# iDC-NEU/NeutronStarLite

Hardware: NVIDIA H100
Metric: gcn_aggregated_edges_per_sec (higher is better)
Workload: dtype f32

## Files before the change

neutronstarlite_b200/csrc/nts_plan.cu:

```cuda
#include <cub/cub.cuh>
#include <cuda_bf16.h>

#include <algorithm>
#include <type_traits>
#include <vector>

#include "nts_common.cuh"

struct nts_gather_plan {
  uint32_t n_rows = 0;
  uint64_t n_edges = 0;
  uint32_t gather_rows = 0;
  int slabs = 1;
  uint32_t slab_rows = 0;
  uint2 *pairs = nullptr;
  uint32_t *voff = nullptr;
  std::vector<uint64_t> slab_edge;
  float *workspace = nullptr;
  size_t workspace_floats = 0;
  __nv_bfloat16 *workspace_bf16 = nullptr;
  size_t workspace_bf16_elems = 0;
  int hub_cols = 0, hub_rows = 0;
  uint32_t *hub_col_ids = nullptr;
  uint32_t *hub_row_ids = nullptr;
  uint32_t lda_c = 0, lda_r = 0;
  float *dense = nullptr;
  size_t dense_floats = 0;
  int last_grid = 0, last_launches = 0, last_k = 0, last_u = 0, last_outv = 0;
  float tuned_ms = 0.f;
};

namespace nts {

static int g_plan_u = 0, g_plan_minb = 0, g_plan_q = 0, g_plan_variant = 0;

__device__ __forceinline__ uint32_t plan_find_row(const uint32_t *__restrict__ off, uint32_t n_rows, uint32_t e) {
  uint32_t lo = 0, hi = n_rows;
  while (hi - lo > 1) {
    uint32_t mid = lo + ((hi - lo) >> 1);
    if (__ldg(off + mid) <= e)
      lo = mid;
    else
      hi = mid;
  }
  return lo;
}

__global__ void plan_keys_kernel(const uint32_t *__restrict__ off, const uint32_t *__restrict__ idx,
                                 const uint32_t *__restrict__ slot_of, uint32_t base, uint32_t n_rows, uint32_t n_edges,
                                 uint32_t slab_rows, uint32_t slabs, uint32_t *__restrict__ key,
                                 uint32_t *__restrict__ val) {
  for (uint64_t e = (uint64_t)blockIdx.x * blockDim.x + threadIdx.x; e < n_edges; e += (uint64_t)gridDim.x * blockDim.x) {
    const uint32_t r = plan_find_row(off, n_rows, (uint32_t)e);
    const uint32_t id = __ldg(idx + e);
    const uint32_t g = slot_of ? __ldg(slot_of + id) : id - base;
    uint32_t s = g / slab_rows;
    if (s >= slabs)
      s = slabs - 1;
    key[e] = s * n_rows + r;
    val[e] = (uint32_t)e;
  }
}

__global__ void plan_pairs_kernel(const uint32_t *__restrict__ perm, const uint32_t *__restrict__ idx,
                                  const float *__restrict__ w, const uint32_t *__restrict__ slot_of, uint32_t base,
                                  uint32_t n_edges, uint2 *__restrict__ pairs) {
  for (uint64_t i = (uint64_t)blockIdx.x * blockDim.x + threadIdx.x; i < n_edges; i += (uint64_t)gridDim.x * blockDim.x) {
    const uint32_t e = perm ? __ldg(perm + i) : (uint32_t)i;
    const uint32_t id = __ldg(idx + e);
    const uint32_t g = slot_of ? __ldg(slot_of + id) : id - base;
    const float wt = w ? __ldg(w + e) : 1.f;
    pairs[i] = make_uint2(g, __float_as_uint(wt));
  }
}

__global__ void plan_part_keys_kernel(const uint32_t *__restrict__ off, const uint32_t *__restrict__ idx,
                                      const uint32_t *__restrict__ slot_of, const float *__restrict__ w, uint32_t base,
                                      uint32_t index_add, uint32_t n_rows_part, uint32_t row_add, uint32_t n_edges,
                                      uint32_t e_off, uint32_t n_rows_total, uint32_t slab_rows, uint32_t slabs,
                                      uint32_t *__restrict__ key, uint32_t *__restrict__ val,
                                      uint2 *__restrict__ unsorted) {
  for (uint64_t e = (uint64_t)blockIdx.x * blockDim.x + threadIdx.x; e < n_edges; e += (uint64_t)gridDim.x * blockDim.x) {
    const uint32_t r = plan_find_row(off, n_rows_part, (uint32_t)e) + row_add;
    const uint32_t id = __ldg(idx + e);
    const uint32_t g = (slot_of ? __ldg(slot_of + id) : id - base) + index_add;
    uint32_t s = g / slab_rows;
    if (s >= slabs)
      s = slabs - 1;
    key[e_off + e] = s * n_rows_total + r;
    val[e_off + e] = e_off + (uint32_t)e;
    unsorted[e_off + e] = make_uint2(g, __float_as_uint(w ? __ldg(w + e) : 1.f));
  }
}
__global__ void plan_permute_pairs_kernel(const uint32_t *__restrict__ perm, const uint2 *__restrict__ unsorted,
                                          uint32_t n_edges, uint2 *__restrict__ pairs) {
  for (uint64_t i = (uint64_t)blockIdx.x * blockDim.x + threadIdx.x; i < n_edges; i += (uint64_t)gridDim.x * blockDim.x)
    pairs[i] = unsorted[__ldg(perm + i)];
}

template <class KeyT>
__global__ void plan_offsets_kernel(const KeyT *__restrict__ sorted_key, uint32_t n_edges, uint32_t n_keys,
                                    uint32_t *__restrict__ voff) {
  for (uint64_t k = (uint64_t)blockIdx.x * blockDim.x + threadIdx.x; k <= n_keys; k += (uint64_t)gridDim.x * blockDim.x) {
    uint32_t lo = 0, hi = n_edges;
    while (lo < hi) {
      uint32_t mid = lo + ((hi - lo) >> 1);
      if (__ldg(sorted_key + mid) < (KeyT)k)
        lo = mid + 1;
      else
        hi = mid;
    }
    voff[k] = lo;
  }
}

constexpr uint32_t kNoHub = 0xffffffffu;

__global__ void plan_ref_count_kernel(const uint32_t *__restrict__ idx, const uint32_t *__restrict__ slot_of,
                                      uint32_t base, uint32_t n_edges, uint32_t *__restrict__ cnt) {
  for (uint64_t e = (uint64_t)blockIdx.x * blockDim.x + threadIdx.x; e < n_edges; e += (uint64_t)gridDim.x * blockDim.x) {
    const uint32_t id = __ldg(idx + e);
    atomicAdd(cnt + (slot_of ? __ldg(slot_of + id) : id - base), 1u);
  }
}

__global__ void plan_hybrid_keys_kernel(const uint32_t *__restrict__ off, const uint32_t *__restrict__ idx,
                                        const uint32_t *__restrict__ slot_of, uint32_t base, uint32_t n_rows,
                                        uint32_t n_edges, uint32_t slab_rows, uint32_t slabs,
                                        const uint32_t *__restrict__ col_slot, const uint32_t *__restrict__ row_slot,
                                        uint32_t lda_c, uint64_t dc_cells, uint32_t lda_r, uint64_t *__restrict__ key,
                                        uint32_t *__restrict__ val) {
  const uint64_t n_keys = (uint64_t)slabs * n_rows;
  for (uint64_t e = (uint64_t)blockIdx.x * blockDim.x + threadIdx.x; e < n_edges; e += (uint64_t)gridDim.x * blockDim.x) {
    const uint32_t r = plan_find_row(off, n_rows, (uint32_t)e);
    const uint32_t id = __ldg(idx + e);
    const uint32_t g = slot_of ? __ldg(slot_of + id) : id - base;
    const uint32_t cs = __ldg(col_slot + g), rs = __ldg(row_slot + r);
    uint64_t k;
    if (cs != kNoHub) {
      k = n_keys + (uint64_t)cs * lda_c + r;
    } else if (rs != kNoHub) {
      k = n_keys + dc_cells + (uint64_t)g * lda_r + rs;
    } else {
      uint32_t s = g / slab_rows;
      if (s >= slabs)
        s = slabs - 1;
      k = (uint64_t)s * n_rows + r;
    }
    key[e] = k;
    val[e] = (uint32_t)e;
  }
}

__global__ void plan_cell_sum_kernel(const uint64_t *__restrict__ cell_key, const uint32_t *__restrict__ run_start,
                                     const uint32_t *__restrict__ run_len, uint32_t n_runs,
                                     const uint32_t *__restrict__ perm, const float *__restrict__ w, uint64_t n_keys,
                                     float *__restrict__ dense) {
  const uint32_t lane = threadIdx.x & 31;
  for (uint64_t run = ((uint64_t)blockIdx.x * blockDim.x + threadIdx.x) >> 5; run < n_runs;
       run += ((uint64_t)gridDim.x * blockDim.x) >> 5) {
    const uint32_t b = __ldg(run_start + run), n = __ldg(run_len + run);
    float s = 0.f;
    for (uint32_t j = lane; j < n; j += 32)
      s += w ? __ldg(w + __ldg(perm + b + j)) : 1.f;
#pragma unroll
    for (int o = 16; o > 0; o >>= 1)
      s += __shfl_xor_sync(0xffffffffu, s, o);
    if (lane == 0)
      dense[__ldg(cell_key + run) - n_keys] = s;
  }
}

__global__ void pad_rows_kernel(const float *__restrict__ src, float *__restrict__ dst, uint32_t n_rows, uint32_t F,
                                uint32_t ld) {
  const uint64_t total = (uint64_t)n_rows * ld;
  for (uint64_t i = (uint64_t)blockIdx.x * blockDim.x + threadIdx.x; i < total; i += (uint64_t)gridDim.x * blockDim.x) {
    const uint64_t r = i / ld;
    const uint32_t c = (uint32_t)(i - r * ld);
    dst[i] = c < F ? __ldg(src + r * F + c) : 0.f;
  }
// ... 337 lines not shown
  auto flush = [&](bool whole) {
    float *orow = out + (size_t)row * F;
#pragma unroll
    for (int k = 0; k < K; k++) {
      const uint32_t col = (c0 + k * 32) * 4;
      if (act[k] && col < F) {
        if (whole)
          flush_chunk<OUTV, false>(orow, col, F, acc[k]);
        else
          flush_chunk<OUTV, true>(orow, col, F, acc[k]);
      }
      acc[k] = make_float4(0.f, 0.f, 0.f, 0.f);
    }
  };
  auto advance = [&](uint32_t ee) {
    flush(row_started_inside);
    do {
      row++;
      row_end = __ldg(off + row + 1);
    } while (ee >= row_end);
    row_started_inside = true;
  };
  if (bulk_bytes)
    p_mbar_wait(bar, 0);
  const uint2 *sp = s_pair - cta_e_base;
  auto issue = [&](uint32_t e, uint32_t stage) {
    const uint32_t src_row = sp[e].x;
    p_mbar_expect_tx(sbar + stage, row_bytes);
    p_bulk_g2s(sbuf + (size_t)stage * tile_vecs, in + (size_t)src_row * ld4 + tile * tile_vecs, row_bytes, sbar + stage);
  };
  if (lane == 0)
    for (uint32_t s = 0; s < STAGES && e0 + s < e1; s++)
      issue(e0 + s, s);
  uint32_t stage = 0, parity = 0;
  for (uint32_t e = e0; e < e1; e++) {
    const float w = __uint_as_float(sp[e].y);
    p_mbar_wait(sbar + stage, parity);
    const float4 *b = sbuf + (size_t)stage * tile_vecs + lane;
    float4 v[K];
#pragma unroll
    for (int k = 0; k < K; k++)
      if (act[k])
        v[k] = b[k * 32];
    if (e >= row_end)
      advance(e);
#pragma unroll
    for (int k = 0; k < K; k++)
      if (act[k]) {
        acc[k].x = fmaf(w, v[k].x, acc[k].x);
        acc[k].y = fmaf(w, v[k].y, acc[k].y);
        acc[k].z = fmaf(w, v[k].z, acc[k].z);
        acc[k].w = fmaf(w, v[k].w, acc[k].w);
      }
    __syncwarp();
    if (lane == 0 && e + STAGES < e1)
      issue(e + STAGES, stage);
    if (++stage == STAGES) {
      stage = 0;
      parity ^= 1u;
    }
  }
  flush(row_started_inside && row_end <= e1);
}

template <int K, int STAGES, int OUTV, int MINB>
static int launch_planned_tma(nts_gather_plan *pl, const PlanShape &sh, const float4 *in, uint32_t ld4, float *out,
                              uint32_t F, uint32_t Q, cudaStream_t st);

struct PlanShape {
  int k, u, outv, minb, g;
  uint32_t tiles, tile_vecs;
};

template <class T, int K, int U, int OUTV, int MINB, int G = 1>
static int launch_planned(nts_gather_plan *pl, const PlanShape &sh, const T *in_rows, uint32_t ldc, float *out,
                          uint32_t F, uint32_t Q, cudaStream_t st) {
  auto kern = planned_gather_sum_kernel<T, K, U, OUTV, MINB, G>;
  const auto *in = reinterpret_cast<const typename GatherT<T>::chunk *>(in_rows);
  const size_t smem = 16 + ((size_t)kPlanWarps * G * Q + 4) * 8;
  NTS_CUDA_OK(cudaFuncSetAttribute(kern, cudaFuncAttributeMaxDynamicSharedMemorySize, (int)smem));
  pl->last_launches = 0;
  for (int s = 0; s < pl->slabs; s++) {
    const uint64_t eb = pl->slab_edge[s], ee = pl->slab_edge[s + 1];
    if (ee <= eb)
      continue;
    const uint64_t quanta = (ee - eb + Q - 1) / Q;
    const uint64_t blocks = (quanta * sh.tiles + kPlanWarps * G - 1) / (kPlanWarps * G);
    NTS_ARG_CHECK(blocks <= 0x7fffffffull, "aggregation grid too large");
    kern<<<(unsigned)blocks, kPlanWarps * 32, smem, st>>>(in, ldc, out, F, pl->pairs, pl->voff + (size_t)s * pl->n_rows,
                                                          pl->n_rows, (uint32_t)eb, (uint32_t)ee, Q, sh.tiles,
                                                          sh.tile_vecs);
    NTS_LAUNCH_CHECK();
    pl->last_grid = (int)blocks;
    pl->last_launches++;
  }
  return 0;
}

template <int K, int STAGES, int OUTV, int MINB>
static int launch_planned_tma(nts_gather_plan *pl, const PlanShape &sh, const float4 *in, uint32_t ld4, float *out,
                              uint32_t F, uint32_t Q, cudaStream_t st) {
  auto kern = planned_gather_sum_tma_kernel<K, STAGES, OUTV, MINB>;
  const uint32_t pair_bytes = (kPlanWarps * Q + 4) * 8;
  const uint32_t ring_bytes = 8u * STAGES + 8u * (STAGES & 1) + STAGES * sh.tile_vecs * 16u;
  const size_t smem = 16 + pair_bytes + (size_t)kPlanWarps * ring_bytes;
  NTS_ARG_CHECK(smem <= 227 * 1024, "row-staging ring does not fit shared memory");
  NTS_CUDA_OK(cudaFuncSetAttribute(kern, cudaFuncAttributeMaxDynamicSharedMemorySize, (int)smem));
  pl->last_launches = 0;
  for (int s = 0; s < pl->slabs; s++) {
    const uint64_t eb = pl->slab_edge[s], ee = pl->slab_edge[s + 1];
    if (ee <= eb)
      continue;
    const uint64_t quanta = (ee - eb + Q - 1) / Q;
    const uint64_t blocks = (quanta * sh.tiles + kPlanWarps - 1) / kPlanWarps;
    NTS_ARG_CHECK(blocks <= 0x7fffffffull, "aggregation grid too large");
    kern<<<(unsigned)blocks, kPlanWarps * 32, smem, st>>>(in, ld4, out, F, pl->pairs, pl->voff + (size_t)s * pl->n_rows,
                                                          pl->n_rows, (uint32_t)eb, (uint32_t)ee, Q, sh.tiles,
                                                          sh.tile_vecs, pair_bytes);
    NTS_LAUNCH_CHECK();
    pl->last_grid = (int)blocks;
    pl->last_launches++;
  }
  return 0;
}

#define NTS_PLAN_TMA_CASE(K_, S_, B_)                                                                               \
  if (sh.k == K_ && stages == S_ && sh.minb == B_) {                                                                \
    if (sh.outv == 4)                                                                                               \
      return launch_planned_tma<K_, S_, 4, B_>(pl, sh, in4, ld4, out, F, Q, st);                                    \
    if (sh.outv == 2)                                                                                               \
      return launch_planned_tma<K_, S_, 2, B_>(pl, sh, in4, ld4, out, F, Q, st);                                    \
    return launch_planned_tma<K_, S_, 1, B_>(pl, sh, in4, ld4, out, F, Q, st);                                      \
  }

#define NTS_PLAN_CASE_G(U_, B_, G_)                                                                                 \
  if (sh.k == 1 && sh.u == U_ && sh.minb == B_ && sh.g == G_) {                                                     \
    if (sh.outv == 4)                                                                                               \
      return launch_planned<T, 1, U_, 4, B_, G_>(pl, sh, in, ldc, out, F, Q, st);                                   \
    if (sh.outv == 2)                                                                                               \
      return launch_planned<T, 1, U_, 2, B_, G_>(pl, sh, in, ldc, out, F, Q, st);                                   \
    return launch_planned<T, 1, U_, 1, B_, G_>(pl, sh, in, ldc, out, F, Q, st);                                     \
  }

#define NTS_PLAN_CASE(K_, U_, B_)                                                                                   \
  if (sh.k == K_ && sh.u == U_ && sh.minb == B_) {                                                                  \
    if (sh.outv == 4)                                                                                               \
      return launch_planned<T, K_, U_, 4, B_>(pl, sh, in, ldc, out, F, Q, st);                                       \
    if (sh.outv == 2)                                                                                               \
      return launch_planned<T, K_, U_, 2, B_>(pl, sh, in, ldc, out, F, Q, st);                                       \
    return launch_planned<T, K_, U_, 1, B_>(pl, sh, in, ldc, out, F, Q, st);                                         \
  }

constexpr int kHubBM = 128, kHubBN = 128, kHubBK = 16, kHubThreads = 256;

__device__ __forceinline__ void p_cp_async16(void *smem_dst, const void *gmem_src, bool full) {
  asm volatile("cp.async.cg.shared.global [%0], [%1], 16, %2;" ::"r"(p_smem_u32(smem_dst)), "l"(gmem_src),
               "r"(full ? 16 : 0)
               : "memory");
}

template <class TB, int OUTV, bool SPLIT>
__global__ void __launch_bounds__(kHubThreads, 2)
    hub_block_gemm_kernel(const float *__restrict__ At, uint32_t lda, uint32_t M, uint32_t K, uint32_t k_split,
                          const TB *__restrict__ B, uint32_t ldb, const uint32_t *__restrict__ colmap,
                          float *__restrict__ out, uint32_t F, const uint32_t *__restrict__ rowmap, uint32_t m_tiles,
                          uint32_t n_tiles) {
  constexpr bool kBf16 = std::is_same<TB, __nv_bfloat16>::value;
  constexpr uint32_t kBV = 16 / sizeof(TB);
  __shared__ __align__(16) float As[2][kHubBK][kHubBM];
  __shared__ __align__(16) TB Bs[2][kHubBK][kHubBN];
  const uint32_t t = threadIdx.x;
  const uint32_t n_tile = blockIdx.x % n_tiles, rest = blockIdx.x / n_tiles;
  const uint32_t m0 = (rest % m_tiles) * kHubBM, n0 = n_tile * kHubBN;
  const uint32_t k_begin = (rest / m_tiles) * k_split;
  const uint32_t k_end = min(K, k_begin + k_split);
  if (k_begin >= k_end)
    return;
  const uint32_t n_kt = (k_end - k_begin + kHubBK - 1) / kHubBK;

  auto load = [&](uint32_t kt, int buf) {
#pragma unroll
    for (int i = 0; i < 2; i++) {
      const uint32_t c = t + i * kHubThreads, kk = c >> 5, c4 = (c & 31) * 4;
      const uint32_t k = k_begin + kt * kHubBK + kk;
      const bool a_ok = k < k_end && m0 + c4 < lda;
      p_cp_async16(&As[buf][kk][c4], a_ok ? At + (size_t)k * lda + m0 + c4 : At, a_ok);
    }
#pragma unroll
    for (int i = 0; i < (int)(kHubBK * kHubBN / kBV / kHubThreads); i++) {
      constexpr uint32_t kRowChunks = kHubBN / kBV;
      const uint32_t c = t + i * kHubThreads, kk = c / kRowChunks, cv = (c % kRowChunks) * kBV;
      const uint32_t k = k_begin + kt * kHubBK + kk;
      const bool b_ok = k < k_end && n0 + cv < ldb;
      const uint32_t brow = b_ok ? (colmap ? __ldg(colmap + k) : k) : 0;
      p_cp_async16(&Bs[buf][kk][cv], B + (size_t)brow * ldb + (b_ok ? n0 + cv : 0), b_ok);
    }
    asm volatile("cp.async.commit_group;" ::: "memory");
  };
  auto read_b4 = [&](int buf, int kk, uint32_t n) -> float4 {
    if constexpr (kBf16) {
      const uint2 u = *reinterpret_cast<const uint2 *>(&Bs[buf][kk][n]);
      return make_float4(__uint_as_float(u.x << 16), __uint_as_float(u.x & 0xffff0000u), __uint_as_float(u.y << 16),
                         __uint_as_float(u.y & 0xffff0000u));
    } else {
      return *reinterpret_cast<const float4 *>(&Bs[buf][kk][n]);
    }
  };

  const uint32_t tx = t & 15, ty = t >> 4;
  float acc[8][8];
#pragma unroll
  for (int i = 0; i < 8; i++)
#pragma unroll
    for (int j = 0; j < 8; j++)
      acc[i][j] = 0.f;

  load(0, 0);
  for (uint32_t kt = 0; kt < n_kt; kt++) {
    const int buf = kt & 1;
    if (kt + 1 < n_kt) {
      load(kt + 1, buf ^ 1);
      asm volatile("cp.async.wait_group 1;" ::: "memory");
    } else {
      asm volatile("cp.async.wait_group 0;" ::: "memory");
    }
    __syncthreads();
#pragma unroll
    for (int kk = 0; kk < kHubBK; kk++) {
      const float4 a0 = *reinterpret_cast<const float4 *>(&As[buf][kk][ty * 4]);
      const float4 a1 = *reinterpret_cast<const float4 *>(&As[buf][kk][64 + ty * 4]);
      const float4 b0 = read_b4(buf, kk, tx * 4);
      const float4 b1 = read_b4(buf, kk, 64 + tx * 4);
      const float a[8] = {a0.x, a0.y, a0.z, a0.w, a1.x, a1.y, a1.z, a1.w};
      const float b[8] = {b0.x, b0.y, b0.z, b0.w, b1.x, b1.y, b1.z, b1.w};
#pragma unroll
      for (int i = 0; i < 8; i++)
#pragma unroll
        for (int j = 0; j < 8; j++)
          acc[i][j] = fmaf(a[i], b[j], acc[i][j]);
    }
    __syncthreads();
  }

#pragma unroll
  for (int i = 0; i < 8; i++) {
    const uint32_t m = m0 + (i >> 2) * 64 + ty * 4 + (i & 3);
    if (m >= M)
      continue;
    float *orow = out + (size_t)(rowmap ? __ldg(rowmap + m) : m) * F;
#pragma unroll
    for (int j = 0; j < 2; j++) {
      const uint32_t col = n0 + j * 64 + tx * 4;
      if (col < F)
        flush_chunk<OUTV, SPLIT>(orow, col, F,
                                 make_float4(acc[i][j * 4], acc[i][j * 4 + 1], acc[i][j * 4 + 2], acc[i][j * 4 + 3]));
    }
  }
}

template <class TB, int OUTV>
static int launch_hub_blocks(nts_gather_plan *pl, const TB *in, uint32_t ldb, float *out, uint32_t F,
                             cudaStream_t st) {
  const uint32_t n_tiles = (F + kHubBN - 1) / kHubBN;
  if (pl->hub_cols) {
    const uint32_t m_tiles = (pl->n_rows + kHubBM - 1) / kHubBM;
    const uint64_t blocks = (uint64_t)m_tiles * n_tiles;
    NTS_ARG_CHECK(blocks <= 0x7fffffffull, "hub column block grid too large");
    hub_block_gemm_kernel<TB, OUTV, false><<<(unsigned)blocks, kHubThreads, 0, st>>>(
        pl->dense, pl->lda_c, pl->n_rows, (uint32_t)pl->hub_cols, (uint32_t)pl->hub_cols, in, ldb, pl->hub_col_ids, out,
        F, nullptr, m_tiles, n_tiles);
    NTS_LAUNCH_CHECK();
  }
  if (pl->hub_rows) {
    const uint32_t m_tiles = (pl->hub_rows + kHubBM - 1) / kHubBM;
    const uint32_t K = pl->gather_rows;
    const uint64_t want = (uint64_t)sm_count() * 2 * 4;
    uint64_t splits = (want + (uint64_t)m_tiles * n_tiles - 1) / ((uint64_t)m_tiles * n_tiles);
    uint32_t k_split = (uint32_t)((K + splits - 1) / splits);
    k_split = std::max<uint32_t>((k_split + kHubBK - 1) / kHubBK * kHubBK, 16 * kHubBK);
    splits = (K + k_split - 1) / k_split;
    hub_block_gemm_kernel<TB, OUTV, true><<<(unsigned)(splits * m_tiles * n_tiles), kHubThreads, 0, st>>>(
        pl->dense + (size_t)pl->hub_cols * pl->lda_c, pl->lda_r, (uint32_t)pl->hub_rows, K, k_split, in, ldb, nullptr,
        out, F, pl->hub_row_ids, m_tiles, n_tiles);
    NTS_LAUNCH_CHECK();
  }
  return 0;
}

template <class T>
static int run_gather(nts_gather_plan *pl, const T *in, uint32_t ld, float *output, uint32_t F, cudaStream_t st) {
  constexpr bool kBf16 = std::is_same<T, __nv_bfloat16>::value;
  PlanShape sh;
  const uint32_t ldc = ld / GatherT<T>::V;
  const uint32_t chunks = (ldc + 31) / 32;
  const uint32_t kmax = 5;
  sh.tiles = (chunks + kmax - 1) / kmax;
  sh.tile_vecs = (ldc + sh.tiles - 1) / sh.tiles;
  sh.k = (int)((sh.tile_vecs + 31) / 32);
  sh.tiles = (ldc + sh.tile_vecs - 1) / sh.tile_vecs;
  sh.outv = (F % 4 == 0 && aligned_to(output, 16)) ? 4 : ((F % 2 == 0 && aligned_to(output, 8)) ? 2 : 1);
  if (pl->hub_cols || pl->hub_rows) {
    const int rc = sh.outv == 4   ? launch_hub_blocks<T, 4>(pl, in, ld, output, F, st)
                   : sh.outv == 2 ? launch_hub_blocks<T, 2>(pl, in, ld, output, F, st)
                                  : launch_hub_blocks<T, 1>(pl, in, ld, output, F, st);
    if (rc)
      return rc;
  }
  sh.g = ldc <= 8 ? 4 : (ldc <= 16 ? 2 : 1);
  if (g_plan_variant == 1 || getenv("NTS_PLAN_NO_SUBWARP"))
    sh.g = 1;
  sh.minb = sh.k >= 3 ? 2 : (sh.k == 2 ? 3 : 4);
  sh.u = sh.k == 4 ? 2 : 4;
  if constexpr (kBf16) {
    sh.minb = sh.k >= 4 ? 2 : (sh.k >= 2 ? 3 : 4);
    sh.u = sh.k == 1 ? 4 : 2;
  }
  {
    static int env_read = 0;
    if (!env_read) {
      env_read = 1;
      if (const char *t = getenv("NTS_PLAN_TUNE"))
        sscanf(t, "%d,%d,%d", &g_plan_u, &g_plan_minb, &g_plan_q);
    }
    if (g_plan_u > 0)
      sh.u = g_plan_u;
    if (g_plan_minb > 0)
      sh.minb = g_plan_minb;
  }
  uint32_t Q = g_plan_q > 0 ? (uint32_t)g_plan_q : 512u / sh.g;
  if (g_plan_q <= 0) {
    const uint64_t per_slab = pl->slab_edge[pl->slabs] / (uint64_t)pl->slabs + 1;
    const uint64_t want_warps = (uint64_t)sm_count() * 64 * sh.g;
    while (Q > 32 && ((per_slab + Q - 1) / Q) * sh.tiles < want_warps)
      Q >>= 1;
  }
  Q = (Q + 31u) & ~31u;
  if (Q * sh.g > 1024)
    Q = (1024 / sh.g) & ~31u;
  pl->last_k = sh.k, pl->last_u = sh.u, pl->last_outv = sh.outv;
  float *out = output;
  if constexpr (kBf16) {
    NTS_PLAN_CASE_G(4, 4, 2)
    NTS_PLAN_CASE_G(4, 4, 4)
    NTS_PLAN_CASE_G(8, 2, 2)
    NTS_PLAN_CASE_G(8, 2, 4)
    if (sh.g != 1)
      return fail(-1, "no BF16 virtual-warp instantiation for this (U, occupancy) point", __FILE__, __LINE__);
    NTS_PLAN_CASE(1, 4, 4)
    NTS_PLAN_CASE(1, 8, 2)
    NTS_PLAN_CASE(2, 2, 3)
    NTS_PLAN_CASE(2, 4, 2)
    NTS_PLAN_CASE(3, 4, 2)
    NTS_PLAN_CASE(3, 2, 3)
    NTS_PLAN_CASE(3, 6, 1)
    NTS_PLAN_CASE(4, 2, 2)
    NTS_PLAN_CASE(4, 4, 2)
    NTS_PLAN_CASE(5, 2, 2)
    return fail(-1, "no BF16 planned-aggregation instantiation for this (chunks, U, occupancy) point", __FILE__,
                __LINE__);
  } else {
  const float4 *in4 = reinterpret_cast<const float4 *>(in);
  const uint32_t ld4 = ldc;
  if (g_plan_variant == 1) {
    const int stages = sh.u >= 8 ? 8 : (sh.u >= 4 ? 4 : 2);
    sh.minb = g_plan_minb > 0 ? g_plan_minb : (sh.k >= 4 ? 2 : 4);
    NTS_PLAN_TMA_CASE(1, 8, 4)
    NTS_PLAN_TMA_CASE(1, 4, 4)
    NTS_PLAN_TMA_CASE(1, 8, 3)
    NTS_PLAN_TMA_CASE(2, 4, 3)
    NTS_PLAN_TMA_CASE(2, 4, 2)
    NTS_PLAN_TMA_CASE(3, 4, 2)
    NTS_PLAN_TMA_CASE(4, 4, 2)
    NTS_PLAN_TMA_CASE(4, 2, 2)
    NTS_PLAN_TMA_CASE(5, 4, 2)
    NTS_PLAN_TMA_CASE(5, 2, 2)
    NTS_PLAN_TMA_CASE(5, 4, 1)
    NTS_PLAN_TMA_CASE(5, 8, 1)
    return fail(-1, "no TMA row-staging instantiation for this (chunks, stages, occupancy) point", __FILE__, __LINE__);
  }
  NTS_PLAN_CASE_G(4, 4, 2)
  NTS_PLAN_CASE_G(4, 4, 4)
  NTS_PLAN_CASE_G(8, 3, 2)
  NTS_PLAN_CASE_G(8, 3, 4)
  if (sh.g != 1)
    return fail(-1, "no virtual-warp instantiation for this (U, occupancy) point", __FILE__, __LINE__);
  NTS_PLAN_CASE(1, 8, 4)
  NTS_PLAN_CASE(1, 4, 4)
  NTS_PLAN_CASE(1, 8, 3)
  NTS_PLAN_CASE(1, 16, 2)
  NTS_PLAN_CASE(2, 4, 3)
  NTS_PLAN_CASE(2, 8, 2)
  NTS_PLAN_CASE(3, 4, 3)
  NTS_PLAN_CASE(3, 4, 2)
  NTS_PLAN_CASE(4, 2, 2)
  NTS_PLAN_CASE(4, 4, 2)
  NTS_PLAN_CASE(5, 2, 2)
  NTS_PLAN_CASE(5, 1, 3)
  NTS_PLAN_CASE(5, 2, 3)
  NTS_PLAN_CASE(5, 4, 1)
  NTS_PLAN_CASE(5, 4, 2)
  return fail(-1, "no planned-aggregation instantiation for this (chunks, U, occupancy) point", __FILE__, __LINE__);
  }
}

template <class E> static int ensure_workspace(E *&ws, size_t &have, size_t elems) {
  if (elems <= have)
    return 0;
  if (ws)
    NTS_CUDA_OK(cudaFree(ws));
  ws = nullptr;
  have = 0;
  NTS_CUDA_OK(cudaMalloc(reinterpret_cast<void **>(&ws), elems * sizeof(E)));
  have = elems;
  return 0;
}

static int run_plan(nts_gather_plan *pl, const float *input, float *output, uint32_t F, cudaStream_t st) {
  if (pl->n_rows == 0 || pl->n_edges == 0 || F == 0)
    return 0;
  NTS_ARG_CHECK(input && output, "null feature pointer");
  const uint32_t ld = (F + 3u) & ~3u;
  const float *in = input;
  if (ld != F || !aligned_to(input, 16)) {
    if (const int rc = ensure_workspace(pl->workspace, pl->workspace_floats, (size_t)pl->gather_rows * ld))
      return rc;
    const uint64_t total = (uint64_t)pl->gather_rows * ld;
    const unsigned blocks = (unsigned)std::min<uint64_t>((total + 255) / 256, (uint64_t)sm_count() * 32);
    pad_rows_kernel<<<blocks, 256, 0, st>>>(input, pl->workspace, pl->gather_rows, F, ld);
    NTS_LAUNCH_CHECK();
    in = pl->workspace;
  }
  return run_gather<float>(pl, in, ld, output, F, st);
}

int to_bf16_rows(const void *src, int dtype, uint32_t lds, void *dst, uint32_t n_rows, uint32_t F, uint32_t ld,
                 cudaStream_t st) {
  NTS_ARG_CHECK(dtype == NTS_DTYPE_F32 || dtype == NTS_DTYPE_BF16, "input dtype must be NTS_DTYPE_F32 or NTS_DTYPE_BF16");
  NTS_ARG_CHECK(ld % 8 == 0 && ld >= F && lds >= F && aligned_to(dst, 16), "bad BF16 row layout");
  if (!n_rows || !F)
    return 0;
  const uint64_t total = (uint64_t)n_rows * (ld / 8);
  const unsigned blocks = (unsigned)std::min<uint64_t>((total + 255) / 256, (uint64_t)sm_count() * 32);
  uint4 *d = static_cast<uint4 *>(dst);
  if (dtype == NTS_DTYPE_F32)
    bf16_rows_kernel<float><<<blocks, 256, 0, st>>>(static_cast<const float *>(src), lds, d, n_rows, F, ld);
  else
    bf16_rows_kernel<__nv_bfloat16><<<blocks, 256, 0, st>>>(static_cast<const __nv_bfloat16 *>(src), lds, d, n_rows,
                                                            F, ld);
  NTS_LAUNCH_CHECK();
  return 0;
}

int run_plan_bf16(nts_gather_plan *pl, const void *input, int dtype, uint32_t lds, float *output, uint32_t F,
                  cudaStream_t st) {
  NTS_ARG_CHECK(dtype == NTS_DTYPE_F32 || dtype == NTS_DTYPE_BF16, "input dtype must be NTS_DTYPE_F32 or NTS_DTYPE_BF16");
  NTS_ARG_CHECK(g_plan_variant == 0, "the TMA row-staging variant (nts_gather_plan_set_variant(1)) gathers FP32 rows only");
  if (pl->n_rows == 0 || pl->n_edges == 0 || F == 0)
    return 0;
  NTS_ARG_CHECK(input && output, "null feature pointer");
  NTS_ARG_CHECK(lds >= F, "row stride below the feature width");
  if (dtype == NTS_DTYPE_BF16 && lds % 8 == 0 && aligned_to(input, 16))
    return run_gather<__nv_bfloat16>(pl, static_cast<const __nv_bfloat16 *>(input), lds, output, F, st);
  const uint32_t ld = (F + 7u) & ~7u;
  if (const int rc = ensure_workspace(pl->workspace_bf16, pl->workspace_bf16_elems, (size_t)pl->gather_rows * ld))
    return rc;
  if (const int rc = to_bf16_rows(input, dtype, lds, pl->workspace_bf16, pl->gather_rows, F, ld, st))
    return rc;
  return run_gather<__nv_bfloat16>(pl, pl->workspace_bf16, ld, output, F, st);
}

}

using namespace nts;

extern "C" {

static int pick_slabs_for_rows(nts_vid_t gather_rows, uint64_t n_edges, nts_vid_t n_rows, uint64_t row_bytes,
                               uint64_t l2_budget_bytes) {
  if (!l2_budget_bytes)
    l2_budget_bytes = 16ull << 20;
  const uint64_t bytes = (uint64_t)gather_rows * row_bytes;
  uint64_t s = (bytes + l2_budget_bytes - 1) / l2_budget_bytes;
  const uint64_t by_degree = n_rows ? n_edges / ((uint64_t)n_rows * 16ull) : 1;
  if (s > by_degree)
    s = by_degree;
  if (s > 64)
    s = 64;
  return s < 1 ? 1 : (int)s;
}

int nts_gather_plan_pick_slabs(nts_vid_t gather_rows, uint64_t n_edges, nts_vid_t n_rows, nts_vid_t feature_size,
                               uint64_t l2_budget_bytes) {
  return pick_slabs_for_rows(gather_rows, n_edges, n_rows, ((feature_size + 3ull) & ~3ull) * 4ull, l2_budget_bytes);
}

static bool hub_counts(const nts_vid_t *offsets, const nts_vid_t *indices, const nts_vid_t *slot_of, nts_vid_t base,
                       uint32_t n_rows, uint32_t E, uint32_t gather_rows, std::vector<uint32_t> &col_cnt,
                       std::vector<uint32_t> &seg, cudaStream_t st) {
  uint32_t *cnt = nullptr;
  std::vector<uint32_t> off(n_rows + 1);
  col_cnt.assign(gather_rows, 0);
  const unsigned blocks = (unsigned)std::min<uint64_t>(((uint64_t)E + 255) / 256, (uint64_t)sm_count() * 32);
  bool ok = cudaMalloc(reinterpret_cast<void **>(&cnt), (size_t)gather_rows * 4) == cudaSuccess &&
            cudaMemsetAsync(cnt, 0, (size_t)gather_rows * 4, st) == cudaSuccess;
  if (ok && E) {
    plan_ref_count_kernel<<<blocks, 256, 0, st>>>(indices, slot_of, base, E, cnt);
    count_launch();
  }
  ok = ok && cudaMemcpyAsync(col_cnt.data(), cnt, (size_t)gather_rows * 4, cudaMemcpyDeviceToHost, st) == cudaSuccess &&
       cudaMemcpyAsync(off.data(), offsets, ((size_t)n_rows + 1) * 4, cudaMemcpyDeviceToHost, st) == cudaSuccess &&
       cudaStreamSynchronize(st) == cudaSuccess;
  cudaFree(cnt);
  seg.resize(n_rows);
  for (uint32_t r = 0; r < n_rows; r++)
    seg[r] = off[r + 1] - off[r];
  return ok;
}

static std::vector<uint32_t> top_ids(const std::vector<uint32_t> &cnt, size_t h) {
  std::vector<uint32_t> ids(cnt.size());
  for (size_t i = 0; i < ids.size(); i++)
    ids[i] = (uint32_t)i;
  h = std::min(h, ids.size());
  std::partial_sort(ids.begin(), ids.begin() + h, ids.end(),
                    [&](uint32_t a, uint32_t b) { return cnt[a] != cnt[b] ? cnt[a] > cnt[b] : a < b; });
  ids.resize(h);
  return ids;
}

static bool build_hybrid(nts_gather_plan *pl, const nts_vid_t *offsets, const nts_vid_t *indices, const float *weight,
                         const nts_vid_t *slot_of, nts_vid_t index_base, int n_hub_cols, int n_hub_rows,
                         cudaStream_t st) {
  const uint32_t E = (uint32_t)pl->n_edges, n_rows = pl->n_rows, G = pl->gather_rows;
  std::vector<uint32_t> col_cnt, seg;
  if (!hub_counts(offsets, indices, slot_of, index_base, n_rows, E, G, col_cnt, seg, st))
    return false;
  const std::vector<uint32_t> cols = top_ids(col_cnt, (size_t)n_hub_cols), rows = top_ids(seg, (size_t)n_hub_rows);
  pl->hub_cols = (int)cols.size();
  pl->hub_rows = (int)rows.size();
  pl->lda_c = (n_rows + 3u) & ~3u;
  pl->lda_r = ((uint32_t)pl->hub_rows + 3u) & ~3u;
  const uint64_t dc_cells = (uint64_t)pl->hub_cols * pl->lda_c;
  pl->dense_floats = dc_cells + (pl->hub_rows ? (uint64_t)G * pl->lda_r : 0);
  std::vector<uint32_t> col_slot(G, kNoHub), row_slot(n_rows, kNoHub);
  for (size_t i = 0; i < cols.size(); i++)
    col_slot[cols[i]] = (uint32_t)i;
  for (size_t i = 0; i < rows.size(); i++)
    row_slot[rows[i]] = (uint32_t)i;

  const uint64_t n_keys = (uint64_t)pl->slabs * n_rows;
  int bits = 1;
  while (bits < 64 && (1ull << bits) < n_keys + pl->dense_floats)
    bits++;
  uint64_t *key_in = nullptr, *key_out = nullptr;
  uint32_t *val_in = nullptr, *val_out = nullptr, *d_col_slot = nullptr, *d_row_slot = nullptr, *d_runs = nullptr;
// ... 193 lines not shown
  if (total >= 0xffffffffull)
    return bad("merged edge count must fit uint32 offsets");
  if (n_slabs < 1 || gather_rows == 0)
    n_slabs = 1;
  if ((uint64_t)n_slabs * n_rows >= 0xffffffffull)
    return bad("slabs * rows must fit 32-bit segment keys");
  nts_gather_plan *pl = new nts_gather_plan();
  pl->n_rows = n_rows;
  pl->n_edges = total;
  pl->gather_rows = gather_rows;
  pl->slabs = n_slabs;
  pl->slab_rows = gather_rows ? (gather_rows + n_slabs - 1) / n_slabs : 1;
  pl->slab_edge.assign(n_slabs + 1, 0);
  if (n_rows == 0 || total == 0)
    return pl;
  const uint32_t E = (uint32_t)total, n_keys = (uint32_t)n_slabs * n_rows;
  uint32_t *key_in = nullptr, *key_out = nullptr, *val_in = nullptr, *val_out = nullptr;
  uint2 *unsorted = nullptr;
  void *tmp = nullptr;
  size_t tmp_bytes = 0;
  int bits = 1;
  while (bits < 32 && (1ull << bits) < (uint64_t)n_keys)
    bits++;
  bool ok = cudaMalloc(reinterpret_cast<void **>(&pl->pairs), (size_t)E * sizeof(uint2)) == cudaSuccess &&
            cudaMalloc(reinterpret_cast<void **>(&pl->voff), ((size_t)n_keys + 1) * sizeof(uint32_t)) == cudaSuccess &&
            cudaMalloc(reinterpret_cast<void **>(&unsorted), (size_t)E * sizeof(uint2)) == cudaSuccess &&
            cudaMalloc(reinterpret_cast<void **>(&key_in), (size_t)E * 4) == cudaSuccess &&
            cudaMalloc(reinterpret_cast<void **>(&key_out), (size_t)E * 4) == cudaSuccess &&
            cudaMalloc(reinterpret_cast<void **>(&val_in), (size_t)E * 4) == cudaSuccess &&
            cudaMalloc(reinterpret_cast<void **>(&val_out), (size_t)E * 4) == cudaSuccess &&
            cub::DeviceRadixSort::SortPairs(nullptr, tmp_bytes, key_in, key_out, val_in, val_out, (int64_t)E, 0, bits, st) ==
                cudaSuccess &&
            cudaMalloc(&tmp, tmp_bytes ? tmp_bytes : 16) == cudaSuccess;
  uint32_t e_off = 0;
  for (int k = 0; k < n_parts && ok; k++) {
    const nts_plan_part &pt = parts[k];
    if (!pt.n_edges)
      continue;
    const unsigned blocks = (unsigned)std::min<uint64_t>((pt.n_edges + 255) / 256, (uint64_t)sm_count() * 32);
    plan_part_keys_kernel<<<blocks, 256, 0, st>>>(pt.offsets, pt.indices, pt.slot_of, pt.weight, pt.index_base,
                                                  pt.index_add, pt.n_rows, pt.row_add, (uint32_t)pt.n_edges, e_off, n_rows,
                                                  pl->slab_rows, (uint32_t)n_slabs, key_in, val_in, unsorted);
    count_launch();
    e_off += (uint32_t)pt.n_edges;
  }
  if (ok)
    ok = cub::DeviceRadixSort::SortPairs(tmp, tmp_bytes, key_in, key_out, val_in, val_out, (int64_t)E, 0, bits, st) ==
         cudaSuccess;
  if (ok) {
    const unsigned blocks = (unsigned)std::min<uint64_t>(((uint64_t)E + 255) / 256, (uint64_t)sm_count() * 32);
    plan_permute_pairs_kernel<<<blocks, 256, 0, st>>>(val_out, unsorted, E, pl->pairs);
    count_launch();
    const unsigned kb = (unsigned)std::min<uint64_t>(((uint64_t)n_keys + 256) / 256, (uint64_t)sm_count() * 32);
    plan_offsets_kernel<uint32_t><<<kb, 256, 0, st>>>(key_out, E, n_keys, pl->voff);
    count_launch();
    std::vector<uint32_t> h(n_slabs + 1);
    ok = cudaStreamSynchronize(st) == cudaSuccess;
    for (int s = 0; s <= n_slabs && ok; s++)
      ok = cudaMemcpy(&h[s], pl->voff + (size_t)s * n_rows, 4, cudaMemcpyDeviceToHost) == cudaSuccess;
    for (int s = 0; s <= n_slabs; s++)
      pl->slab_edge[s] = h[s];
  }
  if (ok)
    ok = cudaStreamSynchronize(st) == cudaSuccess && cudaGetLastError() == cudaSuccess;
  cudaFree(key_in), cudaFree(key_out), cudaFree(val_in), cudaFree(val_out), cudaFree(tmp), cudaFree(unsorted);
  if (!ok) {
    fail(-1, "nts_gather_plan_create_parts: device allocation or preprocessing failed", __FILE__, __LINE__);
    cudaFree(pl->pairs), cudaFree(pl->voff);
    delete pl;
    return nullptr;
  }
  return pl;
}

nts_gather_plan *nts_plan_create_parts_typed(const nts_plan_part *parts, int n_parts, nts_vid_t n_rows,
                                             nts_vid_t gather_rows, int n_slabs, nts_vid_t feature_size, int bf16,
                                             void *stream) {
  if (!parts || n_parts < 1) {
    fail(-1, "no plan parts", __FILE__, __LINE__);
    return nullptr;
  }
  cudaStream_t st = as_stream(stream);
  if (n_slabs >= 1)
    return build_plan_parts(parts, n_parts, n_rows, gather_rows, n_slabs, st);
  uint64_t total = 0;
  for (int k = 0; k < n_parts; k++)
    total += parts[k].n_edges;
  const uint64_t row_bytes = bf16 ? ((feature_size + 7ull) & ~7ull) * 2ull : ((feature_size + 3ull) & ~3ull) * 4ull;
  const int s_max = pick_slabs_for_rows(gather_rows, total, n_rows, row_bytes, 16ull << 20);
  nts_gather_plan *best = build_plan_parts(parts, n_parts, n_rows, gather_rows, 1, st);
  if (!best || s_max <= 1 || total == 0 || feature_size == 0)
    return best;
  float *x = nullptr, *y = nullptr;
  cudaEvent_t e0 = nullptr, e1 = nullptr;
  const size_t xb = (size_t)gather_rows * feature_size * (bf16 ? 2 : sizeof(float)),
               yb = (size_t)n_rows * feature_size * sizeof(float);
  bool ok = cudaMalloc(reinterpret_cast<void **>(&x), xb) == cudaSuccess &&
            cudaMalloc(reinterpret_cast<void **>(&y), yb) == cudaSuccess &&
            cudaMemsetAsync(x, 0, xb, st) == cudaSuccess && cudaMemsetAsync(y, 0, yb, st) == cudaSuccess &&
            cudaEventCreate(&e0) == cudaSuccess && cudaEventCreate(&e1) == cudaSuccess;
  auto time_plan = [&](nts_gather_plan *pl, float *ms) -> bool {
    *ms = 1e30f;
    for (int it = 0; it < 3; it++) {
      float t = 0.f;
      if (cudaEventRecord(e0, st) != cudaSuccess ||
          (bf16 ? run_plan_bf16(pl, x, NTS_DTYPE_BF16, feature_size, y, feature_size, st)
                : run_plan(pl, x, y, feature_size, st)) != 0 ||
          cudaEventRecord(e1, st) != cudaSuccess || cudaEventSynchronize(e1) != cudaSuccess ||
          cudaEventElapsedTime(&t, e0, e1) != cudaSuccess)
        return false;
      if (it > 0 && t < *ms)
        *ms = t;
    }
    return true;
  };
  float best_ms = 0.f;
  ok = ok && time_plan(best, &best_ms);
  for (int s = 2; ok; s *= 2) {
    const int cand = s > s_max ? s_max : s;
    nts_gather_plan *pl = build_plan_parts(parts, n_parts, n_rows, gather_rows, cand, st);
    float ms = 0.f;
    if (!pl || !time_plan(pl, &ms)) {
      nts_gather_plan_destroy(pl);
      break;
    }
    if (ms < best_ms) {
      nts_gather_plan_destroy(best);
      best = pl;
      best_ms = ms;
    } else {
      nts_gather_plan_destroy(pl);
      if (ms > 1.1f * best_ms)
        break;
    }
    if (cand == s_max)
      break;
  }
  cudaFree(x), cudaFree(y);
  if (e0)
    cudaEventDestroy(e0);
  if (e1)
    cudaEventDestroy(e1);
  best->tuned_ms = best_ms;
  return best;
}

nts_gather_plan *nts_gather_plan_create_parts(const nts_plan_part *parts, int n_parts, nts_vid_t n_rows,
                                              nts_vid_t gather_rows, int n_slabs, nts_vid_t feature_size, void *stream) {
  return nts_plan_create_parts_typed(parts, n_parts, n_rows, gather_rows, n_slabs, feature_size, 0, stream);
}

float nts_gather_plan_tuned_ms(const nts_gather_plan *pl) { return pl ? pl->tuned_ms : 0.f; }

static constexpr double kHubFloor = 0.05;
static constexpr int kHubMax = 512;

static nts_gather_plan *create_tuned(const nts_vid_t *offsets, const nts_vid_t *indices, const float *weight,
                                     const nts_vid_t *slot_of, nts_vid_t index_base, nts_vid_t n_rows, uint64_t n_edges,
                                     nts_vid_t gather_rows, nts_vid_t feature_size, bool bf16, void *stream) {
  cudaStream_t st = as_stream(stream);
  const uint64_t row_bytes = bf16 ? ((feature_size + 7ull) & ~7ull) * 2ull : ((feature_size + 3ull) & ~3ull) * 4ull;
  const int s_max = pick_slabs_for_rows(gather_rows, n_edges, n_rows, row_bytes, 16ull << 20);
  const char *hub_env = getenv("NTS_PLAN_HUBS");
  const bool try_hubs = !(hub_env && strcmp(hub_env, "0") == 0) && n_rows > 0 && gather_rows > 0;
  nts_gather_plan *best = nts_gather_plan_create(offsets, indices, weight, slot_of, index_base, n_rows, n_edges,
                                                 gather_rows, 1, stream);
  if (!best || (s_max <= 1 && !try_hubs) || n_edges == 0 || feature_size == 0)
    return best;
  float *x = nullptr, *y = nullptr;
  cudaEvent_t e0 = nullptr, e1 = nullptr;
  const size_t xb = (size_t)gather_rows * feature_size * (bf16 ? 2 : sizeof(float)),
               yb = (size_t)n_rows * feature_size * sizeof(float);
  bool ok = cudaMalloc(reinterpret_cast<void **>(&x), xb) == cudaSuccess &&
            cudaMalloc(reinterpret_cast<void **>(&y), yb) == cudaSuccess &&
            cudaMemsetAsync(x, 0, xb, st) == cudaSuccess && cudaMemsetAsync(y, 0, yb, st) == cudaSuccess &&
            cudaEventCreate(&e0) == cudaSuccess && cudaEventCreate(&e1) == cudaSuccess;
  auto run_one = [&](nts_gather_plan *pl) {
    return bf16 ? run_plan_bf16(pl, x, NTS_DTYPE_BF16, feature_size, y, feature_size, st)
                : run_plan(pl, x, y, feature_size, st);
  };
  auto time_plan = [&](nts_gather_plan *pl, float *ms) -> bool {
    *ms = 1e30f;
    for (int it = 0; it < 3; it++) {
      float t = 0.f;
      if (cudaEventRecord(e0, st) != cudaSuccess || run_one(pl) != 0 ||
          cudaEventRecord(e1, st) != cudaSuccess || cudaEventSynchronize(e1) != cudaSuccess ||
          cudaEventElapsedTime(&t, e0, e1) != cudaSuccess)
        return false;
      if (it > 0 && t < *ms)
        *ms = t;
    }
    return true;
  };
  float best_ms = 0.f;
  ok = ok && time_plan(best, &best_ms);
  auto consider = [&](int s, int hc, int hr, float *ms) -> int {
    nts_gather_plan *pl = nts_gather_plan_create_hybrid(offsets, indices, weight, slot_of, index_base, n_rows, n_edges,
                                                        gather_rows, s, hc, hr, stream);
    if (!pl || !time_plan(pl, ms)) {
      nts_gather_plan_destroy(pl);
      return -1;
    }
    if (*ms < best_ms) {
      nts_gather_plan_destroy(best);
      best = pl;
      best_ms = *ms;
      return 1;
    }
    nts_gather_plan_destroy(pl);
    return 0;
  };
  for (int s = 2; ok && s_max > 1; s *= 2) {
    const int cand = s > s_max ? s_max : s;
    float ms = 0.f;
    const int r = consider(cand, 0, 0, &ms);
    if (r < 0 || (r == 0 && ms > 1.1f * best_ms))
      break;
    if (cand == s_max)
      break;
  }
  if (ok && try_hubs) {
    std::vector<uint32_t> col_cnt, seg;
    ok = hub_counts(offsets, indices, slot_of, index_base, n_rows, (uint32_t)n_edges, gather_rows, col_cnt, seg, st);
    int n_c = 0, n_r = 0;
    for (uint32_t c : col_cnt)
      n_c += c > kHubFloor * n_rows;
    for (uint32_t s : seg)
      n_r += s > kHubFloor * gather_rows;
    const int plain_slabs = best->slabs;
    float ms = 0.f;
    for (int c = 32; ok && c <= std::min(n_c, kHubMax); c *= 2)
      if (consider(best->slabs, c, 0, &ms) != 1)
        break;
    for (int r = 32; ok && r <= std::min(n_r, kHubMax); r *= 2)
      if (consider(best->slabs, best->hub_cols, r, &ms) != 1)
        break;
    if (best->hub_cols || best->hub_rows) {
      const int hc = best->hub_cols, hr = best->hub_rows;
      for (int s : {plain_slabs / 2, std::min(plain_slabs * 2, s_max)})
        if (s >= 1 && s != plain_slabs && s != best->slabs)
          consider(s, hc, hr, &ms);
    }
  }
  cudaFree(x), cudaFree(y);
  if (e0)
    cudaEventDestroy(e0);
  if (e1)
    cudaEventDestroy(e1);
  best->tuned_ms = best_ms;
  return best;
}

nts_gather_plan *nts_gather_plan_create_tuned(const nts_vid_t *offsets, const nts_vid_t *indices, const float *weight,
                                              const nts_vid_t *slot_of, nts_vid_t index_base, nts_vid_t n_rows,
                                              uint64_t n_edges, nts_vid_t gather_rows, nts_vid_t feature_size,
                                              void *stream) {
  return create_tuned(offsets, indices, weight, slot_of, index_base, n_rows, n_edges, gather_rows, feature_size, false,
                      stream);
}

nts_gather_plan *nts_gather_plan_create_tuned_bf16(const nts_vid_t *offsets, const nts_vid_t *indices,
                                                   const float *weight, const nts_vid_t *slot_of, nts_vid_t index_base,
                                                   nts_vid_t n_rows, uint64_t n_edges, nts_vid_t gather_rows,
                                                   nts_vid_t feature_size, void *stream) {
  return create_tuned(offsets, indices, weight, slot_of, index_base, n_rows, n_edges, gather_rows, feature_size, true,
                      stream);
}

int nts_gather_plan_destroy(nts_gather_plan *pl) {
  if (!pl)
    return 0;
  cudaFree(pl->pairs);
  cudaFree(pl->voff);
  cudaFree(pl->workspace);
  cudaFree(pl->workspace_bf16);
  cudaFree(pl->dense);
  cudaFree(pl->hub_col_ids);
  cudaFree(pl->hub_row_ids);
  delete pl;
  return 0;
}

int nts_gather_plan_slabs(const nts_gather_plan *pl) { return pl ? pl->slabs : 0; }

int nts_gather_plan_hubs(const nts_gather_plan *pl, int *cols, int *rows) {
  NTS_ARG_CHECK(pl != nullptr, "null plan");
  if (cols)
    *cols = pl->hub_cols;
  if (rows)
    *rows = pl->hub_rows;
  return 0;
}

uint64_t nts_gather_plan_bytes(const nts_gather_plan *pl) {
  if (!pl)
    return 0;
  return pl->n_edges * 8ull + ((uint64_t)pl->slabs * pl->n_rows + 1) * 4ull + pl->workspace_floats * 4ull +
         pl->workspace_bf16_elems * 2ull + pl->dense_floats * 4ull + ((uint64_t)pl->hub_cols + pl->hub_rows) * 4ull;
}

int nts_gather_plan_last_launch(const nts_gather_plan *pl, int *launches, int *grid, int *k, int *u, int *outv) {
  NTS_ARG_CHECK(pl != nullptr, "null plan");
  if (launches)
    *launches = pl->last_launches;
  if (grid)
    *grid = pl->last_grid;
  if (k)
    *k = pl->last_k;
  if (u)
    *u = pl->last_u;
  if (outv)
    *outv = pl->last_outv;
  return 0;
}

int nts_gather_plan_run(nts_gather_plan *pl, const float *input, float *output, nts_vid_t feature_size, void *stream) {
  NTS_ARG_CHECK(pl != nullptr, "null plan");
  return run_plan(pl, input, output, feature_size, as_stream(stream));
}

int nts_gather_plan_run_bf16(nts_gather_plan *pl, const void *input, int input_dtype, float *output,
                             nts_vid_t feature_size, void *stream) {
  NTS_ARG_CHECK(pl != nullptr, "null plan");
  return run_plan_bf16(pl, input, input_dtype, feature_size, output, feature_size, as_stream(stream));
}

int nts_gather_plan_set_variant(int variant) {
  NTS_ARG_CHECK(variant == 0 || variant == 1, "variant must be 0 (register staging) or 1 (TMA row staging)");
  g_plan_variant = variant;
  return 0;
}

int nts_gather_plan_set_tuning(int u, int min_blocks, int edges_per_warp) {
  NTS_ARG_CHECK(u >= 0 && min_blocks >= 0 && edges_per_warp >= 0 && edges_per_warp <= 4096, "bad tuning point");
  g_plan_u = u;
  g_plan_minb = min_blocks;
  g_plan_q = edges_per_warp;
  return 0;
}

}
```

Before: 14.56 billion.

## Use 3xTF32 tensor-core MMA for hub GEMM, overlap hub rows on side stream

Replaces the FP32 SIMT outer-product inner loop of the hub block GEMM with mma.sync m16n8k8 TF32 instructions, using hi/lo splitting (3xTF32, or 2x for bf16 inputs) to keep near-FP32 accuracy. Shared-memory tiles gain row padding to reduce bank conflicts. The hub-row GEMM now runs on a separate non-blocking stream, forked and joined with events, so it can overlap the sparse gather launches. The hub selection floor and cap are also loosened so more hub columns and rows become dense. The extra MMA passes per tile and the changed stream dependencies add risk.

```diff
diff --git a/neutronstarlite_b200/csrc/nts_plan.cu b/neutronstarlite_b200/csrc/nts_plan.cu
--- a/neutronstarlite_b200/csrc/nts_plan.cu
+++ b/neutronstarlite_b200/csrc/nts_plan.cu
@@ -26,6 +26,9 @@
   uint32_t lda_c = 0, lda_r = 0;
   float *dense = nullptr;
   size_t dense_floats = 0;
+  cudaStream_t row_stream = nullptr;
+  cudaEvent_t row_fork = nullptr, row_join = nullptr;
+  bool row_forked = false;
   int last_grid = 0, last_launches = 0, last_k = 0, last_u = 0, last_outv = 0;
   float tuned_ms = 0.f;
 };
@@ -669,11 +672,24 @@
   }
 
 constexpr int kHubBM = 128, kHubBN = 128, kHubBK = 16, kHubThreads = 256;
+constexpr int kHubLd = 128 + 8;
 
 __device__ __forceinline__ void p_cp_async16(void *smem_dst, const void *gmem_src, bool full) {
   asm volatile("cp.async.cg.shared.global [%0], [%1], 16, %2;" ::"r"(p_smem_u32(smem_dst)), "l"(gmem_src),
                "r"(full ? 16 : 0)
                : "memory");
+}
+
+__device__ __forceinline__ void tf32_split(float x, uint32_t &hi, uint32_t &lo) {
+  hi = (__float_as_uint(x) + 0x1000u) & 0xffffe000u;
+  lo = __float_as_uint(x - __uint_as_float(hi));
+}
+
+__device__ __forceinline__ void mma_tf32(float (&d)[4], const uint32_t (&a)[4], uint32_t b0, uint32_t b1) {
+  asm("mma.sync.aligned.m16n8k8.row.col.f32.tf32.tf32.f32 {%0, %1, %2, %3}, {%4, %5, %6, %7}, {%8, %9}, "
+      "{%0, %1, %2, %3};"
+      : "+f"(d[0]), "+f"(d[1]), "+f"(d[2]), "+f"(d[3])
+      : "r"(a[0]), "r"(a[1]), "r"(a[2]), "r"(a[3]), "r"(b0), "r"(b1));
 }
 
 template <class TB, int OUTV, bool SPLIT>
@@ -684,8 +700,8 @@
                           uint32_t n_tiles) {
   constexpr bool kBf16 = std::is_same<TB, __nv_bfloat16>::value;
   constexpr uint32_t kBV = 16 / sizeof(TB);
-  __shared__ __align__(16) float As[2][kHubBK][kHubBM];
-  __shared__ __align__(16) TB Bs[2][kHubBK][kHubBN];
+  __shared__ __align__(16) float As[2][kHubBK][kHubLd];
+  __shared__ __align__(16) TB Bs[2][kHubBK][kHubLd];
   const uint32_t t = threadIdx.x;
   const uint32_t n_tile = blockIdx.x % n_tiles, rest = blockIdx.x / n_tiles;
   const uint32_t m0 = (rest % m_tiles) * kHubBM, n0 = n_tile * kHubBN;
@@ -714,23 +730,17 @@
     }
     asm volatile("cp.async.commit_group;" ::: "memory");
   };
-  auto read_b4 = [&](int buf, int kk, uint32_t n) -> float4 {
-    if constexpr (kBf16) {
-      const uint2 u = *reinterpret_cast<const uint2 *>(&Bs[buf][kk][n]);
-      return make_float4(__uint_as_float(u.x << 16), __uint_as_float(u.x & 0xffff0000u), __uint_as_float(u.y << 16),
-                         __uint_as_float(u.y & 0xffff0000u));
-    } else {
-      return *reinterpret_cast<const float4 *>(&Bs[buf][kk][n]);
-    }
-  };
-
-  const uint32_t tx = t & 15, ty = t >> 4;
-  float acc[8][8];
-#pragma unroll
-  for (int i = 0; i < 8; i++)
+
+  const uint32_t lane = t & 31, warp = t >> 5, g = lane >> 2, q = lane & 3;
+  const uint32_t wm = (warp & 3) * 32, wn = (warp >> 2) * 64;
+  float acc[2][8][4];
+#pragma unroll
+  for (int i = 0; i < 2; i++)
 #pragma unroll
     for (int j = 0; j < 8; j++)
-      acc[i][j] = 0.f;
+#pragma unroll
+      for (int v = 0; v < 4; v++)
+        acc[i][j][v] = 0.f;
 
   load(0, 0);
   for (uint32_t kt = 0; kt < n_kt; kt++) {
@@ -742,35 +752,60 @@
       asm volatile("cp.async.wait_group 0;" ::: "memory");
     }
     __syncthreads();
-#pragma unroll
-    for (int kk = 0; kk < kHubBK; kk++) {
-      const float4 a0 = *reinterpret_cast<const float4 *>(&As[buf][kk][ty * 4]);
-      const float4 a1 = *reinterpret_cast<const float4 *>(&As[buf][kk][64 + ty * 4]);
-      const float4 b0 = read_b4(buf, kk, tx * 4);
-      const float4 b1 = read_b4(buf, kk, 64 + tx * 4);
-      const float a[8] = {a0.x, a0.y, a0.z, a0.w, a1.x, a1.y, a1.z, a1.w};
-      const float b[8] = {b0.x, b0.y, b0.z, b0.w, b1.x, b1.y, b1.z, b1.w};
-#pragma unroll
-      for (int i = 0; i < 8; i++)
-#pragma unroll
-        for (int j = 0; j < 8; j++)
-          acc[i][j] = fmaf(a[i], b[j], acc[i][j]);
+#pragma unroll 1
+    for (int ks = 0; ks < kHubBK; ks += 8) {
+      uint32_t ahi[2][4], alo[2][4];
+#pragma unroll
+      for (int mi = 0; mi < 2; mi++) {
+        const float *a = &As[buf][ks + q][wm + mi * 16 + g];
+        tf32_split(a[0], ahi[mi][0], alo[mi][0]);
+        tf32_split(a[8], ahi[mi][1], alo[mi][1]);
+        tf32_split(a[4 * kHubLd], ahi[mi][2], alo[mi][2]);
+        tf32_split(a[4 * kHubLd + 8], ahi[mi][3], alo[mi][3]);
+      }
+#pragma unroll
+      for (int ni = 0; ni < 8; ni++) {
+        const uint32_t n = wn + ni * 8 + g;
+        uint32_t bhi0, bhi1, blo0 = 0, blo1 = 0;
+        if constexpr (kBf16) {
+          bhi0 = (uint32_t)reinterpret_cast<const uint16_t &>(Bs[buf][ks + q][n]) << 16;
+          bhi1 = (uint32_t)reinterpret_cast<const uint16_t &>(Bs[buf][ks + q + 4][n]) << 16;
+        } else {
+          tf32_split(Bs[buf][ks + q][n], bhi0, blo0);
+          tf32_split(Bs[buf][ks + q + 4][n], bhi1, blo1);
+        }
+#pragma unroll
+        for (int mi = 0; mi < 2; mi++) {
+          float d[4] = {0.f, 0.f, 0.f, 0.f};
+          mma_tf32(d, alo[mi], bhi0, bhi1);
+          if constexpr (!kBf16)
+            mma_tf32(d, ahi[mi], blo0, blo1);
+          mma_tf32(d, ahi[mi], bhi0, bhi1);
+#pragma unroll
+          for (int v = 0; v < 4; v++)
+            acc[mi][ni][v] += d[v];
+        }
+      }
     }
     __syncthreads();
   }
 
-#pragma unroll
-  for (int i = 0; i < 8; i++) {
-    const uint32_t m = m0 + (i >> 2) * 64 + ty * 4 + (i & 3);
-    if (m >= M)
-      continue;
-    float *orow = out + (size_t)(rowmap ? __ldg(rowmap + m) : m) * F;
-#pragma unroll
-    for (int j = 0; j < 2; j++) {
-      const uint32_t col = n0 + j * 64 + tx * 4;
-      if (col < F)
-        flush_chunk<OUTV, SPLIT>(orow, col, F,
-                                 make_float4(acc[i][j * 4], acc[i][j * 4 + 1], acc[i][j * 4 + 2], acc[i][j * 4 + 3]));
+  uint32_t bid;
+  asm volatile("mov.u32 %0, %%ctaid.x;" : "=r"(bid));
+  const uint32_t em0 = (bid / n_tiles % m_tiles) * kHubBM, en0 = bid % n_tiles * kHubBN;
+  const bool odd = q & 1;
+#pragma unroll
+  for (int mi = 0; mi < 2; mi++) {
+    const uint32_t m = em0 + wm + mi * 16 + g + (odd ? 8 : 0);
+    float *orow = m < M ? out + (size_t)(rowmap ? __ldg(rowmap + m) : m) * F : nullptr;
+#pragma unroll
+    for (int ni = 0; ni < 8; ni++) {
+      const float *c = acc[mi][ni];
+      const float rx = __shfl_xor_sync(0xffffffffu, odd ? c[0] : c[2], 1);
+      const float ry = __shfl_xor_sync(0xffffffffu, odd ? c[1] : c[3], 1);
+      const uint32_t col = en0 + wn + ni * 8 + (q >> 1) * 4;
+      if (orow && col < F)
+        flush_chunk<OUTV, SPLIT>(orow, col, F, odd ? make_float4(rx, ry, c[2], c[3]) : make_float4(c[0], c[1], rx, ry));
     }
   }
 }
@@ -789,6 +824,9 @@
     NTS_LAUNCH_CHECK();
   }
   if (pl->hub_rows) {
+    NTS_CUDA_OK(cudaEventRecord(pl->row_fork, st));
+    NTS_CUDA_OK(cudaStreamWaitEvent(pl->row_stream, pl->row_fork, 0));
+    pl->row_forked = true;
     const uint32_t m_tiles = (pl->hub_rows + kHubBM - 1) / kHubBM;
     const uint32_t K = pl->gather_rows;
     const uint64_t want = (uint64_t)sm_count() * 2 * 4;
@@ -796,7 +834,7 @@
     uint32_t k_split = (uint32_t)((K + splits - 1) / splits);
     k_split = std::max<uint32_t>((k_split + kHubBK - 1) / kHubBK * kHubBK, 16 * kHubBK);
     splits = (K + k_split - 1) / k_split;
-    hub_block_gemm_kernel<TB, OUTV, true><<<(unsigned)(splits * m_tiles * n_tiles), kHubThreads, 0, st>>>(
+    hub_block_gemm_kernel<TB, OUTV, true><<<(unsigned)(splits * m_tiles * n_tiles), kHubThreads, 0, pl->row_stream>>>(
         pl->dense + (size_t)pl->hub_cols * pl->lda_c, pl->lda_r, (uint32_t)pl->hub_rows, K, k_split, in, ldb, nullptr,
         out, F, pl->hub_row_ids, m_tiles, n_tiles);
     NTS_LAUNCH_CHECK();
@@ -805,7 +843,8 @@
 }
 
 template <class T>
-static int run_gather(nts_gather_plan *pl, const T *in, uint32_t ld, float *output, uint32_t F, cudaStream_t st) {
+static int run_gather_launches(nts_gather_plan *pl, const T *in, uint32_t ld, float *output, uint32_t F,
+                               cudaStream_t st) {
   constexpr bool kBf16 = std::is_same<T, __nv_bfloat16>::value;
   PlanShape sh;
   const uint32_t ldc = ld / GatherT<T>::V;
@@ -918,6 +957,22 @@
   NTS_PLAN_CASE(5, 4, 2)
   return fail(-1, "no planned-aggregation instantiation for this (chunks, U, occupancy) point", __FILE__, __LINE__);
   }
+}
+
+template <class T>
+static int run_gather(nts_gather_plan *pl, const T *in, uint32_t ld, float *output, uint32_t F, cudaStream_t st) {
+  if (pl->hub_rows && !pl->row_stream) {
+    NTS_CUDA_OK(cudaStreamCreateWithFlags(&pl->row_stream, cudaStreamNonBlocking));
+    NTS_CUDA_OK(cudaEventCreateWithFlags(&pl->row_fork, cudaEventDisableTiming));
+    NTS_CUDA_OK(cudaEventCreateWithFlags(&pl->row_join, cudaEventDisableTiming));
+  }
+  const int rc = run_gather_launches(pl, in, ld, output, F, st);
+  if (pl->row_forked) {
+    pl->row_forked = false;
+    NTS_CUDA_OK(cudaEventRecord(pl->row_join, pl->row_stream));
+    NTS_CUDA_OK(cudaStreamWaitEvent(st, pl->row_join, 0));
+  }
+  return rc;
 }
 
 template <class E> static int ensure_workspace(E *&ws, size_t &have, size_t elems) {
@@ -1417,8 +1472,8 @@
 
 float nts_gather_plan_tuned_ms(const nts_gather_plan *pl) { return pl ? pl->tuned_ms : 0.f; }
 
-static constexpr double kHubFloor = 0.05;
-static constexpr int kHubMax = 512;
+static constexpr double kHubFloor = 0.035;
+static constexpr int kHubMax = 1024;
 
 static nts_gather_plan *create_tuned(const nts_vid_t *offsets, const nts_vid_t *indices, const float *weight,
                                      const nts_vid_t *slot_of, nts_vid_t index_base, nts_vid_t n_rows, uint64_t n_edges,
@@ -1535,6 +1590,12 @@
 int nts_gather_plan_destroy(nts_gather_plan *pl) {
   if (!pl)
     return 0;
+  if (pl->row_stream) {
+    cudaStreamSynchronize(pl->row_stream);
+    cudaStreamDestroy(pl->row_stream);
+    cudaEventDestroy(pl->row_fork);
+    cudaEventDestroy(pl->row_join);
+  }
   cudaFree(pl->pairs);
   cudaFree(pl->voff);
   cudaFree(pl->workspace);
```

Measured after the change: 15.09 billion (median of 6 runs). +3.7%, better.
